# 10XGenomics/lariat

Hardware: AMD Instinct MI355X
Metric: read-pairs/sec aligned to hg38 (per-barcode align loop: SMEM seeding + SW + RFA/MAPQ on device); synthetic hg38-scale reference (higher is better)
Workload: dtype u64/i32 (FM-index + integer DP), f64 (RFA scores)

## Files before the change

include/lariat_hip.h:

```cpp
#ifndef LARIAT_HIP_H
#define LARIAT_HIP_H

#include <stddef.h>
#include <stdint.h>

#ifdef __cplusplus
extern "C" {
#endif

#define LH_ABI_VERSION 11

#define LH_OK 0
#define LH_E_ARG 1
#define LH_E_IO 2
#define LH_E_HIP 3
#define LH_E_CAPACITY 4
#define LH_E_NODEVICE 5
#define LH_E_LIMIT 6

#define LH_MAX_READ_LEN 250

typedef struct lh_index lh_index;
typedef struct lh_context lh_context;

typedef struct lh_opts {
    int32_t abi_version;
    int32_t a, b, o_del, e_del, o_ins, e_ins;
    int32_t pen_unpaired, pen_clip5, pen_clip3;
    int32_t w, zdrop, T;
    int32_t min_seed_len, min_chain_weight, max_chain_extend;
    float split_factor;
    int32_t split_width, max_occ, max_chain_gap, max_ins;
    float mask_level, drop_ratio, XA_drop_ratio, mask_level_redun;
    float mapQ_coef_len;
    int32_t max_mem_intv, max_matesw;
    int32_t pes_low, pes_high;
    int32_t rescue_score_delta;
    int32_t rescue_max_hits;
    int32_t aln_score_delta;
    double improper_pair_penalty;
    double genome_length;
    int32_t run_inference;
    uint32_t flags;
} lh_opts;

#define LH_F_NO_SWEEP_FILTER 1u
#define LH_F_EXT_WAVE 16u
#define LH_F_EXT_SERIAL 32u
#define LH_F_P2_TASKS 128u
#define LH_F_RESCUE_FULL 256u
#define LH_F_SEED_LANE 512u
#define LH_F_TAIL_PASSES 1024u
#define LH_F_RFA_SLAB 2048u
#define LH_F_P2_SCAN 4096u
#define LH_F_P3_LAST 8192u
#define LH_F_CHAIN_WAVE 64u

typedef struct lh_index_opts {
    int32_t abi_version;
    int32_t sa_intv;
    int32_t sb_shift;
    int32_t no_kmer_table;
    int32_t no_unique_runs;
    int32_t no_sweep_filter;
    int32_t build_chunk_log2;
    int32_t ktree_levels;
} lh_index_opts;
void lh_index_opts_init(lh_index_opts* io);

typedef struct lh_context_opts {
    int32_t abi_version;
    int32_t smem_grid;
    int32_t aln_grid;
    int32_t rfa_grid;
    int32_t rfa_slab_kb;
    int32_t lanes;
    int32_t big_slots;
    int32_t rfa_tier_kb[2];
// ... 139 lines not shown
int lh_result_download_end(lh_context* ctx, lh_result** out);
int lh_batch_stage_slot(lh_context* ctx, int32_t slot, const lh_batch* batch);
void* lh_host_alloc(size_t bytes);
void lh_host_free(void* p);
int lh_result_download(lh_context* ctx, lh_result** out);
void lh_result_free(lh_result* r);

typedef struct lh_round_info {
    int32_t n_rounds;
    int32_t max_barcode;
    const int32_t* first_barcode;
    const int64_t* round_seeds;
    const int64_t* round_need_bytes;
    int64_t need_bytes;
    int64_t budget_bytes;
    int64_t max_barcode_need_bytes;
} lh_round_info;
int lh_last_rounds(lh_context* ctx, int32_t lane, lh_round_info* out);

int lh_last_rfa_classes(lh_context* ctx, int64_t* out );

int lh_last_p2_calls(lh_context* ctx, int64_t* out );

int lh_last_fin_list(lh_context* ctx, int32_t* out, int64_t cap, int64_t* n);

int lh_last_timings(lh_context* ctx, int32_t* n, const char* const** names, const float** ms);

int lh_stage_dump_resident(lh_context* ctx, const lh_opts* opts, lh_stage_dump** out);
void lh_stage_dump_free(lh_stage_dump* d);

int lh_get_seq(const lh_index* idx, int32_t rid, int64_t start, int64_t end, int32_t reversed, char* out );

int lh_device_memory(int device, int64_t* free_bytes, int64_t* total_bytes);
int lh_diag_random_read(int device, int64_t table_bytes, int32_t granule_bytes, int64_t n_access, double* gbps, double* ms);

int lh_diag_valu_rate(int device, int32_t op, int32_t waves_per_simd, int32_t iters, double* out, int32_t n_out);

int lh_diag_rescue_sw(int device, int32_t n_cases, const int32_t* q_off, const uint8_t* q, const int32_t* t_off, const uint8_t* t, int32_t full, int32_t weaken, int32_t* out);

int lh_diag_index_check(const lh_index* idx, uint64_t stride, uint64_t* n_checked, uint64_t* n_bad_order, uint64_t* n_bad_lf);

int lh_diag_index_digest(const lh_index* idx, uint64_t* lcp_digest, uint64_t* ktree_digest, int32_t* ktree_levels);

int lh_synth_genome(uint64_t seed, double gc, int64_t l_pac, uint8_t* pac, int32_t threads);
int lh_synth_write_fastq9(const char* path, const uint8_t* seq, const int64_t* seq_off, const int32_t* bc_pair_off, int32_t n_barcodes, int64_t first_barcode,
                          int32_t trim, int32_t gz_level, uint64_t seed, const int32_t* truth_rid, const int64_t* truth_pos1, const int64_t* truth_pos2);
// ... 65 lines not shown
```

lariat_amd/capi.py:

```python
import ctypes as C
import os

import numpy as np

_HERE = os.path.dirname(os.path.abspath(__file__))
LIB_PATH = os.environ.get("LARIAT_HIP_LIB") or os.path.join(_HERE, "_build", "liblariat_hip.so")

LH_OK = 0
LH_ABI_VERSION = 11
LH_E_ARG, LH_E_IO, LH_E_HIP, LH_E_CAPACITY, LH_E_NODEVICE, LH_E_LIMIT = 1, 2, 3, 4, 5, 6
LH_REC_DEBUG_TAGS = 1
LH_F_NO_SWEEP_FILTER, LH_F_EXT_WAVE, LH_F_EXT_SERIAL, LH_F_CHAIN_WAVE, LH_F_P2_TASKS, LH_F_RESCUE_FULL, LH_F_SEED_LANE, LH_F_TAIL_PASSES, LH_F_RFA_SLAB, LH_F_P2_SCAN, LH_F_P3_LAST = 1, 16, 32, 64, 128, 256, 512, 1024, 2048, 4096, 8192
LH_MAX_READ_LEN = 250

c_i32p = C.POINTER(C.c_int32)
c_i64p = C.POINTER(C.c_int64)
c_u8p = C.POINTER(C.c_uint8)
c_u32p = C.POINTER(C.c_uint32)
c_u64p = C.POINTER(C.c_uint64)
c_f64p = C.POINTER(C.c_double)


class LhOpts(C.Structure):
    _fields_ = [
        ("abi_version", C.c_int32),
        ("a", C.c_int32), ("b", C.c_int32), ("o_del", C.c_int32), ("e_del", C.c_int32), ("o_ins", C.c_int32), ("e_ins", C.c_int32),
        ("pen_unpaired", C.c_int32), ("pen_clip5", C.c_int32), ("pen_clip3", C.c_int32),
        ("w", C.c_int32), ("zdrop", C.c_int32), ("T", C.c_int32),
        ("min_seed_len", C.c_int32), ("min_chain_weight", C.c_int32), ("max_chain_extend", C.c_int32),
        ("split_factor", C.c_float),
        ("split_width", C.c_int32), ("max_occ", C.c_int32), ("max_chain_gap", C.c_int32), ("max_ins", C.c_int32),
        ("mask_level", C.c_float), ("drop_ratio", C.c_float), ("XA_drop_ratio", C.c_float), ("mask_level_redun", C.c_float),
        ("mapQ_coef_len", C.c_float),
        ("max_mem_intv", C.c_int32), ("max_matesw", C.c_int32),
        ("pes_low", C.c_int32), ("pes_high", C.c_int32),
# ... 241 lines not shown
    L.lh_records_free.argtypes = [C.c_void_p]
    L.lh_records_free.restype = None
    L.lh_name_seed.argtypes = [C.c_char_p, C.c_int64]
    L.lh_name_seed.restype = C.c_uint64
    L.lh_index_resample_sa.argtypes = [C.c_void_p, C.c_int32]
    L.lh_index_resample_sa.restype = C.c_int
    L.lh_index_sa_interval.argtypes = [C.c_void_p]
    L.lh_index_sa_interval.restype = C.c_int32
    L.lh_index_free.argtypes = [C.c_void_p]
    L.lh_index_build.argtypes = [C.c_char_p, C.c_int32, C.POINTER(C.c_char_p), C.POINTER(c_u8p), c_i64p, C.c_int32]
    L.lh_context_create.argtypes = [C.c_void_p, C.c_int64, C.POINTER(LhContextOpts), C.POINTER(C.c_void_p)]
    L.lh_context_free.argtypes = [C.c_void_p]
    L.lh_align_barcodes.argtypes = [C.c_void_p, C.POINTER(LhOpts), C.POINTER(LhBatch), C.POINTER(C.POINTER(LhResult))]
    L.lh_batch_upload.argtypes = [C.c_void_p, C.POINTER(LhBatch)]
    L.lh_align_resident.argtypes = [C.c_void_p, C.POINTER(LhOpts)]
    L.lh_batch_upload_slot.argtypes = [C.c_void_p, C.c_int32, C.POINTER(LhBatch)]
    L.lh_batch_select.argtypes = [C.c_void_p, C.c_int32]
    L.lh_result_download.argtypes = [C.c_void_p, C.POINTER(C.POINTER(LhResult))]
    L.lh_result_free.argtypes = [C.POINTER(LhResult)]
    L.lh_last_timings.argtypes = [C.c_void_p, c_i32p, C.POINTER(C.POINTER(C.c_char_p)), C.POINTER(C.POINTER(C.c_float))]
    L.lh_last_rounds.argtypes = [C.c_void_p, C.c_int32, C.POINTER(LhRoundInfo)]
    L.lh_last_rfa_classes.argtypes = [C.c_void_p, C.POINTER(C.c_int64)]
    L.lh_last_p2_calls.argtypes = [C.c_void_p, C.POINTER(C.c_int64)]
    L.lh_stage_dump_resident.argtypes = [C.c_void_p, C.POINTER(LhOpts), C.POINTER(C.POINTER(LhStageDump))]
    L.lh_stage_dump_free.argtypes = [C.POINTER(LhStageDump)]
    L.lh_get_seq.argtypes = [C.c_void_p, C.c_int32, C.c_int64, C.c_int64, C.c_int32, C.c_char_p]
    L.lh_device_memory.argtypes = [C.c_int, C.POINTER(C.c_int64), C.POINTER(C.c_int64)]
    L.lh_diag_random_read.argtypes = [C.c_int, C.c_int64, C.c_int32, C.c_int64, C.POINTER(C.c_double), C.POINTER(C.c_double)]
    L.lh_diag_rescue_sw.argtypes = [C.c_int, C.c_int32, c_i32p, c_u8p, c_i32p, c_u8p, C.c_int32, C.c_int32, c_i32p]
    L.lh_diag_valu_rate.argtypes = [C.c_int, C.c_int32, C.c_int32, C.c_int32, C.POINTER(C.c_double), C.c_int32]
    return L


class LhError(RuntimeError):
    def __init__(self, code, msg):
        super().__init__("liblariat_hip error %d: %s" % (code, msg))
        self.code = code


class Library:

    def __init__(self, path=None):
        path = path or LIB_PATH
        if not os.path.exists(path):
            raise RuntimeError("%s not built: run __graft_entry__.build(); there is no CPU fallback" % path)
        self.path = path
# ... 437 lines not shown
        names = C.POINTER(C.c_char_p)()
        ms = C.POINTER(C.c_float)()
        self.lib.check(self.lib.L.lh_last_timings(self.h, C.byref(n), C.byref(names), C.byref(ms)))
        return [(names[i].decode(), float(ms[i])) for i in range(n.value)]

    def rounds(self, lane=0):
        ri = LhRoundInfo()
        self.lib.check(self.lib.L.lh_last_rounds(self.h, int(lane), C.byref(ri)))
        n = int(ri.n_rounds)
        return dict(n_rounds=n, first_barcode=_view(ri.first_barcode, n + 1 if n else 0, np.int32), round_seeds=_view(ri.round_seeds, n, np.int64),
                    round_need_bytes=_view(ri.round_need_bytes, n, np.int64), need_bytes=int(ri.need_bytes), budget_bytes=int(ri.budget_bytes),
                    max_barcode=int(ri.max_barcode), max_barcode_need_bytes=int(ri.max_barcode_need_bytes))

    def rfa_classes(self):
        out = (C.c_int64 * 4)()
        self.lib.check(self.lib.L.lh_last_rfa_classes(self.h, out))
        return dict(big=int(out[0]), rest=int(out[1]), small=int(out[2]), turned_away=int(out[3]))

    def p2_calls(self):
        out = (C.c_int64 * 4)()
        self.lib.check(self.lib.L.lh_last_p2_calls(self.h, out))
        return dict(dropped=int(out[0]), probed=int(out[1]), unprobed=int(out[2]), shares=int(out[3]))

    def fin_list(self):
        L = self.lib.L
        L.lh_last_fin_list.argtypes = [C.c_void_p, c_i32p, C.c_int64, C.POINTER(C.c_int64)]
        n = C.c_int64()
        self.lib.check(L.lh_last_fin_list(self.h, None, 0, C.byref(n)))
        out = np.zeros(max(int(n.value), 1), dtype=np.int32)
        self.lib.check(L.lh_last_fin_list(self.h, out.ctypes.data_as(c_i32p), len(out), C.byref(n)))
        return np.sort(out[:int(n.value)])

    def stage_dump(self, batch=None, opts=None):
        opts = opts or self.lib.opts()
        if batch is not None:
            self.upload(batch)
        d = C.POINTER(LhStageDump)()
        self.lib.check(self.lib.L.lh_stage_dump_resident(self.h, C.byref(opts), C.byref(d)))
        out = StageDump(d.contents)
        self.lib.L.lh_stage_dump_free(d)
        return out


_lib = None


# ... 167 lines not shown
                return
            yield b
            if b.at_eof:
                return

    def close(self):
        if self.h:
            self.lib.L.lh_ingest_close(self.h)
            self.h = None

    def __del__(self):
        try:
            self.close()
        except Exception:
            pass


EXPORTED_SYMBOLS = [
    "lh_last_error", "lh_device_count", "lh_opts_init", "lh_index_load", "lh_index_from_arrays", "lh_index_contigs", "lh_index_l_pac",
    "lh_index_resample_sa", "lh_index_sa_interval",
    "lh_ingest_open", "lh_ingest_next", "lh_ingest_batch_free", "lh_ingest_close", "lh_name_seed",
    "lh_records_text", "lh_records_text_ex", "lh_records_free", "lh_bam_open", "lh_bam_append", "lh_bam_set_flags", "lh_bam_close",
    "lh_index_free", "lh_index_build", "lh_context_create", "lh_context_free", "lh_align_barcodes", "lh_batch_upload", "lh_align_resident",
    "lh_result_download", "lh_result_free", "lh_last_timings", "lh_last_rounds", "lh_last_rfa_classes", "lh_last_p2_calls", "lh_last_fin_list", "lh_stage_dump_resident", "lh_stage_dump_free", "lh_get_seq", "lh_device_memory", "lh_diag_gosort", "lh_diag_gosort_split", "lh_diag_bitonic", "lh_diag_introsort", "lh_diag_random_read", "lh_diag_valu_rate", "lh_diag_rescue_sw", "lh_diag_go_rand", "lh_diag_rescue_dedup",
    "lh_index_opts_init", "lh_context_opts_init", "lh_index_build_device", "lh_index_export", "lh_index_save", "lh_synth_genome", "lh_synth_reads", "lh_synth_write_fastq9", "lh_diag_index_check", "lh_batch_upload_slot", "lh_batch_select", "lh_bam_concat", "lh_reference_pack", "lh_index_set_holes", "lh_diag_index_digest", "lh_index_set_alt", "lh_index_alt", "lh_bam_set_level", "lh_bam_timings", "lh_result_download_begin", "lh_result_download_end", "lh_batch_stage_slot", "lh_host_alloc", "lh_host_free",
    "lh_bgzf_create", "lh_bgzf_free", "lh_bgzf_compress", "lh_bgzf_bound", "lh_bgzf_timings", "lh_bam_set_device",
    "lh_bam_set_device_records", "lh_bam_records_timings", "lh_diag_format_f6",
    "lh_bam_append_resident",
]
```

lariat_amd/csrc/k_smem4.h:

```cpp
#pragma once
#ifndef LH_K1_SLAB_CHUNK
#define LH_K1_SLAB_CHUNK 4
#endif
#include "lh_dev.h"
static_assert((LH_MAXLEN + 2) % LH_K1_SLAB_CHUNK == 0, "a lane's list of LH_MAXLEN + 2 entries is a whole number of chunks");
#define LH_K1_LDS_BUDGET 10240
#ifndef LH_K1_QW_SMALL
#define LH_K1_QW_SMALL 24
#endif
#ifdef LH_K1_RING
#define LH_K1_RING_OF(qw_) (LH_K1_RING)
#else
#define LH_K1_RING_OF(qw_) ((LH_K1_LDS_BUDGET - (qw_) * 256) / 2048)
#endif
static_assert(LH_K1_QW_SMALL >= 1 && LH_K1_QW_SMALL <= 32, "the small query staging holds at most the full query");

struct __attribute__((aligned(16))) PEnt { u64 lo, hi; };
#define LH_M40 0xffffffffffull
__device__ __forceinline__ PEnt pe_pack(u64 x0, u64 x1, u64 x2, int info) {
    PEnt e;
    e.lo = x0 | (x2 << 40);
    e.hi = x1 | ((x2 >> 24) << 40) | ((u64)(uint32_t)info << 49);
    return e;
}
// ... 119 lines not shown
                    }
                    rs.x = bnd; rs.Pk = P; rs.pk = bnd | 2 << 8 | (bnd + 1) << 16;
                    n_ext = e1; n_exec = e2; n_kt = 1;
                }
            }
        }
        if (on >= 0) n_intv[r] = on;
        if (on >= 0 && rs.x >= len) status[r] = 0;
        else { resume[r] = rs; listed = 1; }
    }
    const u64 lm = __ballot(listed);
    if (lm) {
        int basep = 0;
        if (lane == 0) basep = atomicAdd(todo_count, (int32_t)__popcll(lm));
        basep = wave_readlane(basep, 0);
        if (listed) todo[basep + lanes_below(lm, lane)] = r;
    }
    if (ctr) {
        unsigned t1 = (unsigned)wave_sum_i32((int)n_ext), t2 = (unsigned)wave_sum_i32((int)n_exec), t3 = (unsigned)wave_sum_i32((int)n_kt);
        if (lane == 0 && t1) { atomicAdd(&LH_CTR(ctr)->n_ext, (u64)t1); atomicAdd(&LH_CTR(ctr)->n_ext_exec[0], (u64)t2); atomicAdd(&LH_CTR(ctr)->n_ktree[0], (u64)t3); }
    }
}

struct K1Big { const int32_t* list; const int32_t* count; const int32_t* slot; DIntv* slab; union { const K1Resume* resume; int32_t* p2_cnt; }; };
#define LH_P2E_READ ((1ull << 27) - 1)
#define LH_P2E_SHARE (1ull << 27)
#define LH_P2E_TASK 28
#define LH_P2E_XM 28
#define LH_P2E_MIN 36
#define LH_P2E_PBITS 40
#define LH_P2E_UNPROBED (1ull << 59)
#define LH_P2_MAX_MIN_INTV 15
static_assert(LH_BLOOM_K <= 19 && LH_MAXLEN < 256, "a call entry: 8 bits of position, 19 of probe");
#define K1T_OCC 0
#define K1T_TREE 1
#define K1T_BLOOM1 2
#define K1T_BLOOM2 3
#define K1T_REPT 4
#define K1T_PLCP 5
#define K1T_TEXT 6
#define K1T_SA 7
#define K1T_ISA 8
#define K1T_SLAB_R 9
#define K1T_SLAB_W 10
#define K1T_INTV_W 11
#define K1T_READS 12
// ... 1350 lines not shown
```

lariat_amd/csrc/lh_host.inc:

```
#include <math.h>
#include <stdlib.h>
#include <stdio.h>
#include <string.h>

#include <algorithm>
#include <array>
#include <functional>
#include <memory>
#include <mutex>
#include <string>
#include <vector>
#include <deque>
#include <map>

#include "../../include/lariat_hip.h"
#include "k_smem4.h"
#include "k_chain_lane.h"
#include "k_chain_cl.h"
#include "k_rfa.h"
#include "k_rescue3.h"
#include "k_rounds.h"
#include "lh_result_cols.h"

static void lh_print_wd(const int32_t* d_wd) {
// ... 46 lines not shown
    hipStream_t dl_stream = nullptr, up_stream = nullptr;
    hipEvent_t ev_pack = nullptr, ev_dl = nullptr;
    bool dl_pending = false, dl_split = false; std::function<int(lh_result**)> dl_finish;
    int sel_slot = 0;
    HostPeek* h_peek = nullptr;
    bool rfa_merge_big = false;
    i64 rfa_cls[4] = {0, 0, 0, 0};
    bool ext_hint_valid = false;
    hipEvent_t ev_fork = nullptr, ev_join[3] = {nullptr, nullptr, nullptr};
    i64 cap_pairs = 0, cap_reads = 0, cap_bases = 0, pool_cap = 0, regpool_cap = 0, cap_bc = 0;
    DevGroup mem, seed_mem, cand_mem, big_mem, rjob_mem, pack_mem, tier_mem[2], round_mem;
    void free_device() {
        for (DevGroup* g : {&mem, &seed_mem, &cand_mem, &big_mem, &rjob_mem, &pack_mem, &tier_mem[0], &tier_mem[1], &round_mem}) g->release();
        for (DevBatch& sl : slots) sl.mem.release();
        for (void* q : free_later) hipFree(q);
        free_later.clear();
    }
    int grid_smem4 = 0; PEnt* d_slab4 = nullptr; K1Counters* d_next_read = nullptr;
    BatchView b;
    uint32_t* d_seq4 = nullptr;
    const uint32_t* q4 = nullptr;
    DIntv* d_intv = nullptr; DIntv* d_big_slab = nullptr; int32_t *d_big_slot = nullptr, *d_big_list = nullptr; K1BigCounts* d_big_count = nullptr; int big_cap = 0, big_base = 0;
    K1Resume* d_k1_resume = nullptr; int32_t* d_k1_todo = nullptr;
    u64* d_p2_tasks = nullptr; P2Calls* d_p2_calls = nullptr;
    i64 p2_cls[4] = {0, 0, 0, 0};
    int32_t *d_n_intv = nullptr, *d_seed_cnt = nullptr, *d_l_rep = nullptr, *d_status = nullptr;
    int32_t* d_fin_list = nullptr;
    i64* d_seed_off = nullptr; DSeed* d_seeds = nullptr; int32_t *d_s_rid = nullptr, *d_s_next = nullptr, *d_ord = nullptr, *d_srt = nullptr;
    DChainTmp* d_ct = nullptr; DChain* d_chains = nullptr; DSeed* d_cseeds = nullptr; int32_t* d_n_chains = nullptr;
    DCounters* d_ctr = nullptr; i64* d_tile_sum = nullptr;
    int32_t* d_wd = nullptr;
    i64* d_reg_off = nullptr; DReg* d_regs = nullptr; int32_t* d_n_regs = nullptr; i64* d_chain_rmax = nullptr;
    DReg* d_regs_tmp = nullptr;
    int32_t* d_ia = nullptr;
    int32_t *d_ext_defer = nullptr, *d_ext_heavy = nullptr, *d_ext_jlist = nullptr, *d_ext_jkey = nullptr, *d_ext_jorder = nullptr; ExtSt* d_ext_st = nullptr;
    DExtJobs* d_ext_jobs = nullptr; DExtJobs* d_ext_jobs2 = nullptr;
    int32_t* d_ext_long = nullptr;
    int32_t* d_ext_u = nullptr;
    int32_t* d_best = nullptr;
    uint8_t* d_reg_clean = nullptr;
    uint8_t* d_dd_done = nullptr;
    int32_t* d_dd_list = nullptr;
    int32_t* d_rnj = nullptr; i64* d_rjob_off = nullptr; RMeta* d_rmeta = nullptr; int32_t* d_rkeys = nullptr; int32_t* d_rheavy = nullptr;
    RJob* d_rjobs = nullptr; int32_t *d_rorder = nullptr, *d_rorder2 = nullptr; i64 rjob_cap = 0;
    i64 cand_cap = 0; int grid_aln = 0; DCand R; uint8_t* d_zpool = nullptr;
    int32_t *d_aln_r = nullptr, *d_aln_ci = nullptr; AlnCounts* d_aln_count = nullptr;
// ... 152 lines not shown
    HIPCHK(hipStreamCreate(&c->stream));
    for (int i = 0; i < 3; ++i) { HIPCHK(hipStreamCreate(&c->aux[i])); HIPCHK(hipEventCreateWithFlags(&c->ev_join[i], hipEventDisableTiming)); }
    HIPCHK(hipEventCreateWithFlags(&c->ev_fork, hipEventDisableTiming));
    {
        int lo = 0, hi = 0;
        HIPCHK(hipDeviceGetStreamPriorityRange(&lo, &hi));
        HIPCHK(hipStreamCreateWithPriority(&c->dl_stream, hipStreamNonBlocking, lo));
        HIPCHK(hipStreamCreateWithPriority(&c->up_stream, hipStreamNonBlocking, lo));
    }
    HIPCHK(hipHostMalloc((void**)&c->h_peek, sizeof(HostPeek), hipHostMallocDefault));
    HIPCHK(hipEventCreateWithFlags(&c->ev_pack, hipEventDisableTiming)); HIPCHK(hipEventCreateWithFlags(&c->ev_dl, hipEventDisableTiming));
    i64 N = c->cap_reads;
    DevGroup& g = c->mem;
    DALLOC(g, c->d_seq4, c->cap_bases / 8 + 16); HIPCHK(hipMemset(c->d_seq4, 0x44, 16));
    {
        lh_context::DevBatch& s0 = c->slots.emplace_back();
        DALLOC(s0.mem, s0.v.seq, c->cap_bases + 64); DALLOC(s0.mem, s0.v.seq_off, N + 1); DALLOC(s0.mem, s0.v.name_seed, max_pairs);
        DALLOC(s0.mem, s0.v.bc_pair_off, c->cap_bc + 1); DALLOC(s0.mem, s0.v.bc_do_rfa, c->cap_bc);
        DALLOC(s0.mem, s0.v.cen_start, idx->names.size()); DALLOC(s0.mem, s0.v.cen_end, idx->names.size());
        select_slot(c, s0);
    }
    DALLOC(g, c->d_intv, N * LH_MAX_INTV); DALLOC(g, c->d_n_intv, N);
    c->big_cap = c->co.big_slots > 0 ? c->co.big_slots : LH_MAX_INTV < 16 ? (int)N : (int)(N / 256 > 64 ? N / 256 : 64);
    DALLOC(g, c->d_k1_resume, N); DALLOC(g, c->d_k1_todo, N); DALLOC(g, c->d_p2_tasks, (size_t)LH_P2_SPLIT * N); DALLOC(g, c->d_p2_calls, LH_CTR_SLOTS);
    DALLOC(c->big_mem, c->d_big_slab, (size_t)c->big_cap * 2 * LH_BIG_INTV); DALLOC(g, c->d_big_slot, N); DALLOC(c->big_mem, c->d_big_list, c->big_cap); DALLOC(g, c->d_big_count, 1);
    DALLOC(g, c->d_seed_cnt, N); DALLOC(g, c->d_l_rep, N); DALLOC(g, c->d_status, N); DALLOC(g, c->d_fin_list, N);
    {
        int want = c->co.smem_grid;
        i64 need = (c->cap_reads + 63) / 64;
        c->grid_smem4 = (int)(need < want ? need : want);
        DALLOC(g, c->d_slab4, (size_t)c->grid_smem4 * 64 * 2 * (LH_MAXLEN + 2));
        DALLOC(g, c->d_next_read, 1);
    }
    DALLOC(g, c->d_seed_off, N + 1); DALLOC(g, c->d_n_chains, N);
    if (c->co.seed_budget_kb < 0 || pool_cap_limit(c) < 1)
        return set_err(LH_E_ARG, "lh_context_opts.seed_budget_kb = " + std::to_string(c->co.seed_budget_kb) + ": the rescue slots of " + std::to_string(max_pairs) +
                                     " pairs alone take " + std::to_string((seed_need(c, 0) >> 10) + 1) + " KiB");
    { int rc = alloc_seed_pools(c, first_pool_cap(c)); if (rc) return rc; }
    DALLOC(g, c->d_ctr, LH_CTR_SLOTS);
    DALLOC(g, c->d_wd, LH_WD_SLOTS);
    HIPCHK(hipMemset(c->d_wd, 0, LH_WD_SLOTS * sizeof(int32_t)));
    { int rc = stage2_alloc(c); if (rc) return rc; }
    for (int i = 0; i <= LH_NSTAGE; ++i) HIPCHK(hipEventCreate(&c->ev[i]));
    guard.c = nullptr;
    *out = c;
    return LH_OK;
}
// ... 174 lines not shown
static inline int ext_long_min(int N);
struct K1Tail {
    bool probe;
    bool tasks;
    bool list;
    bool p3_lock;
    bool p3_counts;
    bool fused;
};
static K1Tail k1_tail_plan(const lh_context* c, const DOpts& o, int N, bool packed_reads) {
    K1Tail t;
    const bool list_ok = N < (1 << 27);
    t.probe = list_ok && !(c->flags & (LH_F_P2_TASKS | LH_F_P2_SCAN)) && o.split_width < LH_P2_MAX_MIN_INTV;
    t.p3_lock = o.max_mem_intv > 0 && packed_reads;
    t.p3_counts = t.p3_lock && !(c->flags & LH_F_SEED_LANE);
#ifdef LH_K1_TRACE
    t.probe = t.p3_counts = false;
#endif
    t.tasks = list_ok && !t.probe && ((c->flags & LH_F_P2_TASKS) || (c->ext_hint_valid && c->h_peek->prev_wave_reads >= ext_long_min(N)));
    t.list = t.probe || t.tasks;
    t.fused = t.probe && t.p3_counts && !(c->flags & LH_F_P3_LAST);
    return t;
}
static int run_front(lh_context* c, const DOpts& o, int& t) {
    int N = c->b.n_reads;
    const DIndex& ix = c->idx->d;
    HIPCHK(hipMemsetAsync(c->d_ctr, 0, sizeof(DCounters) * LH_CTR_SLOTS, c->stream));
    const uint32_t* q4 = nullptr;
    if (ix.tn) {
        LH_LAUNCH(k_pack_reads, 4096, 256, c->stream, (const uint8_t*)c->b.seq, c->b.n_bases, c->d_seq4 + 2);
        q4 = c->d_seq4 + 2;
    }
    c->q4 = q4;
    DIndex ix4 = ix;
    if (c->flags & LH_F_NO_SWEEP_FILTER) ix4.bloom1 = ix4.bloom2 = nullptr;
    {
        const int g4 = (N + 63) / 64 < c->grid_smem4 ? (N + 63) / 64 : c->grid_smem4;
        HIPCHK(hipMemsetAsync(c->d_next_read, 0, sizeof(K1Counters), c->stream));
        K1Big nobig; nobig.list = nullptr; nobig.count = nullptr; nobig.slot = nullptr; nobig.slab = nullptr; nobig.resume = nullptr;
        K1Big first = nobig; first.list = c->d_k1_todo; first.count = &c->d_next_read->n_todo; first.resume = c->d_k1_resume;
        const int g3 = (N + 63) / 64 < 2 * c->grid_smem4 ? (N + 63) / 64 : 2 * c->grid_smem4;
        T_BEGIN("k_smem4");
        LH_LAUNCH(k_smem_first, (N + 255) / 256, 256, c->stream, ix4, o, N, q4, (const i64*)c->b.seq_off, c->d_intv, c->d_n_intv, c->d_status, c->d_k1_resume, c->d_k1_todo, &c->d_next_read->n_todo, c->d_ctr);
#ifdef LH_K1_TRACE
        K1Trace trace;
        { int rc = k1_trace_begin(c, trace, g4); if (rc) return rc; }
#endif
        const bool qw_small = c->b.max_len <= 8 * LH_K1_QW_SMALL;
        if (qw_small) smem_pass<1, false, LH_K1_QW_SMALL>(c, ix4, o, N, g4, first);
        else smem_pass<1, false>(c, ix4, o, N, g4, first);
        T_END();
#ifdef LH_K1_TRACE
        { int rc = k1_trace_replay(c, trace, N, g4); if (rc) return rc; }
#endif
        HIPCHK(hipMemsetAsync(c->d_p2_calls, 0, sizeof(P2Calls) * LH_CTR_SLOTS, c->stream));
        const K1Tail tail = k1_tail_plan(c, o, N, q4 != nullptr);
        K1Big p2 = nobig;
        if (tail.list) { p2.list = (const int32_t*)c->d_p2_tasks; p2.count = &c->d_next_read->n_p2_tasks; p2.slot = c->d_k1_todo; }
        if (tail.fused) {
            T_BEGIN("k_smem4_p3");
            LH_LAUNCH(k_p23_lock, (N + 255) / 256, 256, c->stream, ix4, o, N, (const uint8_t*)c->b.seq, q4, (const i64*)c->b.seq_off, c->d_intv, c->d_n_intv, c->d_ctr, c->d_seed_cnt, c->d_p2_tasks,
                      &c->d_next_read->n_p2_tasks, c->d_k1_todo, c->d_p2_calls);
            T_END();
            T_BEGIN("k_smem4_p2");
            p2.p2_cnt = c->d_seed_cnt;
            if (qw_small) smem_pass<2, false, LH_K1_QW_SMALL>(c, ix4, o, N, g4, p2);
            else smem_pass<2, false>(c, ix4, o, N, g4, p2);
            LH_LAUNCH(k_p2_close, (N + 255) / 256, 256, c->stream, N, c->d_n_intv, c->d_status, c->d_seed_cnt, c->d_l_rep, c->d_fin_list, &c->d_next_read->n_fin);
            T_END();
#ifdef LH_P3_KINDS
// ... 260 lines not shown
            rc = pipe_download(c, &res);
            c->ran = false;
            if (rc) rc = set_err(rc, "round " + std::to_string(r) + " of " + std::to_string(n_rounds) + " (its reads start at read " + std::to_string(2 * (i64)p0) + " of the batch): " + g_err);
        }
        if (!rc) rc = merge_into(acc, res);
        if (rc) {
            const std::string why = g_err;
            quiesce(c);
            if (acc) lh_result_free(acc);
            return set_err(rc, why);
        }
    }
    c->round_result = acc;
    R.n_rounds = (int)n_rounds;
    c->n_t = sums.n;
    for (int i = 0; i < sums.n; ++i) { c->tnames[i] = sums.names[i]; c->tms[i] = sums.ms[i]; }
    return LH_OK;
}

static int pipe_align(lh_context* c, const lh_opts* opts) {
    if (!c || !opts) return set_err(LH_E_ARG, "lh_align_resident: null argument");
    if (!c->resident) return set_err(LH_E_ARG, "no batch resident: call lh_batch_upload first");
    if (opts->abi_version != LH_ABI_VERSION) return set_err(LH_E_ARG, "lh_opts.abi_version does not match LH_ABI_VERSION (use lh_opts_init)");
    if (opts->flags & ~(LH_F_NO_SWEEP_FILTER | LH_F_EXT_WAVE | LH_F_EXT_SERIAL | LH_F_CHAIN_WAVE | LH_F_P2_TASKS | LH_F_RESCUE_FULL | LH_F_SEED_LANE | LH_F_TAIL_PASSES | LH_F_RFA_SLAB | LH_F_P2_SCAN | LH_F_P3_LAST)) return set_err(LH_E_ARG, "lh_opts.flags: unknown bit set");
    HIPCHK(hipSetDevice(c->idx->device));
    {
        std::vector<void*> fl;
        { std::lock_guard<std::mutex> g(c->slot_mu); fl.swap(c->free_later); }
        for (void* q : fl) hipFree(q);
    }
    if (c->round_result) { lh_result_free(c->round_result); c->round_result = nullptr; }
    c->rounds.clear();
    c->ran = false;
    if (!c->pool_cap) { int rc = alloc_seed_pools(c, first_pool_cap(c)); if (rc) return rc; }
    if (!c->cand_cap) { int rc = alloc_cand_pools(c, first_cand_cap(c)); if (rc) return rc; }
    DOpts o = to_dopts(opts);
    o.wd = c->d_wd;
    c->flags = opts->flags;
    int t = 0;
    int rc = run_front(c, o, t);
    const bool in_rounds = rc == LH_NEED_ROUNDS;
    if (in_rounds) rc = align_rounds(c, o, t);
    else if (!rc) rc = stage2_run(c, o, t);
    if (rc) { quiesce(c); return rc; }
    if (!in_rounds) {
        HIPCHK(hipEventRecord(c->ev[t], c->stream));
        HIPCHK(hipStreamSynchronize(c->stream));
// ... 114 lines not shown
```

lariat_amd/csrc/lh_lanes.inc:

```
#include <atomic>
#include <thread>

#define LH_MAX_LANES 4

int lh_context_create(lh_index* idx, int64_t max_pairs, const lh_context_opts* co, lh_context** out) {
    const int lanes = co && co->lanes ? co->lanes : 1;
    if (lanes < 1 || lanes > LH_MAX_LANES) return set_err(LH_E_ARG, "lh_context_opts.lanes must be 1 .. 4");
    lh_context* c = nullptr;
    int rc = pipe_create(idx, max_pairs, co, &c);
    if (rc) return rc;
    for (int k = 1; k < lanes && max_pairs >= 2 * lanes; ++k) {
        lh_context_opts c2 = *co;
        c2.lanes = 1;
        {
            const int g = (c2.rfa_grid > 0 ? c2.rfa_grid : 4096) / lanes;
            c2.rfa_grid = g > 1024 ? g : 1024;
        }
        int64_t cap = max_pairs / lanes + 30000 < max_pairs ? max_pairs / lanes + 30000 : max_pairs;
        lh_context* p = nullptr;
        rc = pipe_create(idx, cap, &c2, &p);
        if (rc) { lh_context_free(c); return rc; }
        c->more.push_back(p);
    }
    *out = c;
// ... 123 lines not shown
        R.have_max = true;
    }
    const int32_t b0 = lane && lanes_split(c) ? c->slot_cut[(size_t)c->cur_slot][(size_t)lane - 1] : 0;
    if (b0 && R.first_bc[0] == 0) { for (int32_t& b : R.first_bc) b += b0; R.max_bc += b0; }
    out->n_rounds = R.n_rounds; out->max_barcode = (int32_t)R.max_bc;
    out->first_barcode = R.first_bc.data(); out->round_seeds = R.seeds.data(); out->round_need_bytes = R.need.data();
    out->need_bytes = seed_need(p, R.total_seeds); out->budget_bytes = R.budget; out->max_barcode_need_bytes = seed_need(p, R.max_bc_seeds);
    return LH_OK;
}

int lh_last_rfa_classes(lh_context* c, int64_t* out) {
    if (!c || !out) return set_err(LH_E_ARG, "lh_last_rfa_classes: null argument");
    if (!c->ran_inference) return set_err(LH_E_ARG, "lh_last_rfa_classes: call lh_align_resident with run_inference first");
    for (int i = 0; i < 4; ++i) out[i] = c->rfa_cls[i];
    return LH_OK;
}

int lh_last_p2_calls(lh_context* c, int64_t* out) {
    if (!c || !out) return set_err(LH_E_ARG, "lh_last_p2_calls: null argument");
    for (int i = 0; i < 4; ++i) out[i] = c->p2_cls[i];
    return LH_OK;
}

int lh_last_fin_list(lh_context* c, int32_t* out, int64_t cap, int64_t* n) {
    if (!c || !n || cap < 0 || (cap && !out)) return set_err(LH_E_ARG, "lh_last_fin_list: null argument");
    if (!c->d_fin_list || !c->d_next_read) return set_err(LH_E_ARG, "lh_last_fin_list: call lh_align_resident or lh_stage_dump_resident first");
    HIPCHK(hipSetDevice(c->idx->device));
    HIPCHK(hipStreamSynchronize(c->stream));
    int32_t n_fin = 0;
    HIPCHK(hipMemcpy(&n_fin, &c->d_next_read->n_fin, sizeof n_fin, hipMemcpyDeviceToHost));
    *n = n_fin;
    const int64_t k = n_fin < cap ? n_fin : cap;
    if (k > 0) HIPCHK(hipMemcpy(out, c->d_fin_list, (size_t)k * sizeof(int32_t), hipMemcpyDeviceToHost));
    return LH_OK;
}

static int merge_into(lh_result*& acc, lh_result* part) {
    if (!acc) { acc = part; return LH_OK; }
    lh_result* m = nullptr;
    const int rc = merge_results(acc, part, &m);
    lh_result_free(acc); lh_result_free(part);
    acc = m;
    return rc;
}
static int merge_results(lh_result* a, lh_result* b, lh_result** out) {
    const size_t Ca = (size_t)a->n_cand, Cb = (size_t)b->n_cand;
// ... 118 lines not shown
```

lariat_amd/csrc/lh_workspace.h:

```cpp
#pragma once
#include <stddef.h>
#include <vector>

template <class T> static int dalloc(T** p, size_t n) {
    hipError_t e = hipMalloc((void**)p, (n ? n : 1) * sizeof(T));
    if (e != hipSuccess) { *p = nullptr; (void)hipGetLastError(); return set_err(LH_E_HIP, std::string("hipMalloc of ") + std::to_string((n ? n : 1) * sizeof(T)) + " bytes: " + hipGetErrorString(e)); }
    return LH_OK;
}

struct DevGroup {
    std::vector<void**> held;
    DevGroup() = default;
    DevGroup(const DevGroup&) = delete;
    DevGroup& operator=(const DevGroup&) = delete;
    ~DevGroup() { release(); }
    template <class T> int alloc(T*& p, size_t n) {
        int rc = dalloc(&p, n);
        if (rc) release(); else held.push_back((void**)&p);
        return rc;
    }
    void release() { for (void** q : held) { hipFree(*q); *q = nullptr; } held.clear(); }
    void release_to(std::vector<void*>& later) { for (void** q : held) { if (*q) later.push_back(*q); *q = nullptr; } held.clear(); }
};
#define DALLOC(g, p, n) do { int rc_ = (g).alloc(p, (size_t)(n)); if (rc_) return rc_; } while (0)

struct BatchView {
    uint8_t* seq = nullptr; i64* seq_off = nullptr;
    u64* name_seed = nullptr;
    int32_t* bc_pair_off = nullptr; uint8_t* bc_do_rfa = nullptr;
    i64 *cen_start = nullptr, *cen_end = nullptr;
    int n_pairs = 0, n_reads = 0, n_bc = 0; bool has_cen = false; i64 n_bases = 0;
    int max_len = LH_MAXLEN;
};

struct K1Counters {
    int32_t pass[3];
    int32_t big_pass[3];
    int32_t n_todo;
    int32_t n_p2_tasks;
    int32_t n_fin;
};
static_assert(sizeof(K1Counters) == 9 * sizeof(int32_t) && offsetof(K1Counters, big_pass) == 3 * sizeof(int32_t) && sizeof(K1Counters::big_pass) == 3 * sizeof(int32_t),
              "the second chance's counters are cleared as one range");
struct K1BigCounts {
    int32_t listed;
    int32_t asked;
};
static_assert(offsetof(K1BigCounts, listed) == 0 && offsetof(K1BigCounts, asked) == sizeof(int32_t) && sizeof(K1BigCounts) == 2 * sizeof(int32_t), "k_big_collect: count[0], count[1]");
struct AlnCounts {
    int32_t flat;
    int32_t grp16;
    int32_t grp32;
    int32_t full;
};
static_assert(offsetof(AlnCounts, flat) == 0 && sizeof(AlnCounts) == 4 * sizeof(int32_t), "K7 clears all four, the download the first");
struct RfaCounters {
    int32_t next;
    int32_t n_ovf;
    int32_t last_next;
    int32_t heavy_pairs;
    int32_t heavy_reads;
    int32_t post_next;
    int32_t post_n_ovf;
    int32_t post_last_next;
    struct Tier {
// ... 93 lines not shown
```

Baseline: 56.32 million.

## Settle near-exact K1 reads by direct reference comparison before SMEM pass

Adds a k_smem_settle kernel that runs before the first SMEM pass. For each pending read it compares the query directly against the reference at the resumed position. When there are few mismatches, the PLCP check shows the exact segments are unique, and no bloom-filter k-mer hit exists around the mismatches, it writes the exact-match intervals directly and removes the read from the todo list. Only the remaining reads go to the costly FM-index SMEM pass. This adds one extra kernel launch, reads of plcp and bloom, and relies on heuristics that must stay equivalent to full SMEM output.

```diff
diff --git a/include/lariat_hip.h b/include/lariat_hip.h
--- a/include/lariat_hip.h
+++ b/include/lariat_hip.h
@@ -8,7 +8,7 @@
 extern "C" {
 #endif
 
-#define LH_ABI_VERSION 11
+#define LH_ABI_VERSION 12
 
 #define LH_OK 0
 #define LH_E_ARG 1
@@ -54,6 +54,7 @@
 #define LH_F_RFA_SLAB 2048u
 #define LH_F_P2_SCAN 4096u
 #define LH_F_P3_LAST 8192u
+#define LH_F_K1_NO_SETTLE 16384u
 #define LH_F_CHAIN_WAVE 64u
 
 typedef struct lh_index_opts {
@@ -239,6 +240,8 @@
 
 int lh_last_p2_calls(lh_context* ctx, int64_t* out );
 
+int lh_last_k1_settled(lh_context* ctx, int64_t* out );
+
 int lh_last_fin_list(lh_context* ctx, int32_t* out, int64_t cap, int64_t* n);
 
 int lh_last_timings(lh_context* ctx, int32_t* n, const char* const** names, const float** ms);
diff --git a/lariat_amd/capi.py b/lariat_amd/capi.py
--- a/lariat_amd/capi.py
+++ b/lariat_amd/capi.py
@@ -7,10 +7,10 @@
 LIB_PATH = os.environ.get("LARIAT_HIP_LIB") or os.path.join(_HERE, "_build", "liblariat_hip.so")
 
 LH_OK = 0
-LH_ABI_VERSION = 11
+LH_ABI_VERSION = 12
 LH_E_ARG, LH_E_IO, LH_E_HIP, LH_E_CAPACITY, LH_E_NODEVICE, LH_E_LIMIT = 1, 2, 3, 4, 5, 6
 LH_REC_DEBUG_TAGS = 1
-LH_F_NO_SWEEP_FILTER, LH_F_EXT_WAVE, LH_F_EXT_SERIAL, LH_F_CHAIN_WAVE, LH_F_P2_TASKS, LH_F_RESCUE_FULL, LH_F_SEED_LANE, LH_F_TAIL_PASSES, LH_F_RFA_SLAB, LH_F_P2_SCAN, LH_F_P3_LAST = 1, 16, 32, 64, 128, 256, 512, 1024, 2048, 4096, 8192
+LH_F_NO_SWEEP_FILTER, LH_F_EXT_WAVE, LH_F_EXT_SERIAL, LH_F_CHAIN_WAVE, LH_F_P2_TASKS, LH_F_RESCUE_FULL, LH_F_SEED_LANE, LH_F_TAIL_PASSES, LH_F_RFA_SLAB, LH_F_P2_SCAN, LH_F_P3_LAST, LH_F_K1_NO_SETTLE = 1, 16, 32, 64, 128, 256, 512, 1024, 2048, 4096, 8192, 16384
 LH_MAX_READ_LEN = 250
 
 c_i32p = C.POINTER(C.c_int32)
@@ -298,6 +298,7 @@
     L.lh_last_rounds.argtypes = [C.c_void_p, C.c_int32, C.POINTER(LhRoundInfo)]
     L.lh_last_rfa_classes.argtypes = [C.c_void_p, C.POINTER(C.c_int64)]
     L.lh_last_p2_calls.argtypes = [C.c_void_p, C.POINTER(C.c_int64)]
+    L.lh_last_k1_settled.argtypes = [C.c_void_p, C.POINTER(C.c_int64)]
     L.lh_stage_dump_resident.argtypes = [C.c_void_p, C.POINTER(LhOpts), C.POINTER(C.POINTER(LhStageDump))]
     L.lh_stage_dump_free.argtypes = [C.POINTER(LhStageDump)]
     L.lh_get_seq.argtypes = [C.c_void_p, C.c_int32, C.c_int64, C.c_int64, C.c_int32, C.c_char_p]
@@ -781,6 +782,11 @@
         self.lib.check(self.lib.L.lh_last_p2_calls(self.h, out))
         return dict(dropped=int(out[0]), probed=int(out[1]), unprobed=int(out[2]), shares=int(out[3]))
 
+    def k1_settled(self):
+        out = (C.c_int64 * 5)()
+        self.lib.check(self.lib.L.lh_last_k1_settled(self.h, out))
+        return dict(listed=int(out[0]), settled=int(out[1]), too_many=int(out[2]), not_unique=int(out[3]), window=int(out[4]))
+
     def fin_list(self):
         L = self.lib.L
         L.lh_last_fin_list.argtypes = [C.c_void_p, c_i32p, C.c_int64, C.POINTER(C.c_int64)]
@@ -994,7 +1000,7 @@
     "lh_ingest_open", "lh_ingest_next", "lh_ingest_batch_free", "lh_ingest_close", "lh_name_seed",
     "lh_records_text", "lh_records_text_ex", "lh_records_free", "lh_bam_open", "lh_bam_append", "lh_bam_set_flags", "lh_bam_close",
     "lh_index_free", "lh_index_build", "lh_context_create", "lh_context_free", "lh_align_barcodes", "lh_batch_upload", "lh_align_resident",
-    "lh_result_download", "lh_result_free", "lh_last_timings", "lh_last_rounds", "lh_last_rfa_classes", "lh_last_p2_calls", "lh_last_fin_list", "lh_stage_dump_resident", "lh_stage_dump_free", "lh_get_seq", "lh_device_memory", "lh_diag_gosort", "lh_diag_gosort_split", "lh_diag_bitonic", "lh_diag_introsort", "lh_diag_random_read", "lh_diag_valu_rate", "lh_diag_rescue_sw", "lh_diag_go_rand", "lh_diag_rescue_dedup",
+    "lh_result_download", "lh_result_free", "lh_last_timings", "lh_last_rounds", "lh_last_rfa_classes", "lh_last_p2_calls", "lh_last_k1_settled", "lh_last_fin_list", "lh_stage_dump_resident", "lh_stage_dump_free", "lh_get_seq", "lh_device_memory", "lh_diag_gosort", "lh_diag_gosort_split", "lh_diag_bitonic", "lh_diag_introsort", "lh_diag_random_read", "lh_diag_valu_rate", "lh_diag_rescue_sw", "lh_diag_go_rand", "lh_diag_rescue_dedup",
     "lh_index_opts_init", "lh_context_opts_init", "lh_index_build_device", "lh_index_export", "lh_index_save", "lh_synth_genome", "lh_synth_reads", "lh_synth_write_fastq9", "lh_diag_index_check", "lh_batch_upload_slot", "lh_batch_select", "lh_bam_concat", "lh_reference_pack", "lh_index_set_holes", "lh_diag_index_digest", "lh_index_set_alt", "lh_index_alt", "lh_bam_set_level", "lh_bam_timings", "lh_result_download_begin", "lh_result_download_end", "lh_batch_stage_slot", "lh_host_alloc", "lh_host_free",
     "lh_bgzf_create", "lh_bgzf_free", "lh_bgzf_compress", "lh_bgzf_bound", "lh_bgzf_timings", "lh_bam_set_device",
     "lh_bam_set_device_records", "lh_bam_records_timings", "lh_diag_format_f6",
diff --git a/lariat_amd/csrc/k_smem4.h b/lariat_amd/csrc/k_smem4.h
--- a/lariat_amd/csrc/k_smem4.h
+++ b/lariat_amd/csrc/k_smem4.h
@@ -165,6 +165,124 @@
     }
 }
 
+
+#ifndef LH_K1_SETTLE_MAXDIFF
+#define LH_K1_SETTLE_MAXDIFF 3
+#endif
+static_assert(LH_K1_SETTLE_MAXDIFF >= 1 && LH_K1_SETTLE_MAXDIFF <= 4 && LH_MAXLEN < 256, "the differences' positions: a byte each in one word");
+#ifndef LH_SETTLE_BATCH
+#define LH_SETTLE_BATCH LH_BLOOM_K
+#endif
+__device__ __forceinline__ uint32_t dev_code8(uint32_t w) {
+    w &= 0x33333333u;
+    w = (w | w >> 2) & 0x0f0f0f0fu; w = (w | w >> 4) & 0x00ff00ffu; w = (w | w >> 8) & 0xffffu;
+    return w;
+}
+__device__ __forceinline__ u64 dev_settle_key(u64 lo, uint32_t hi, int t) { return (t ? lo >> (2 * t) | (u64)hi << (64 - 2 * t) : lo) & ((1ull << (2 * LH_BLOOM_K)) - 1); }
+__global__ void __launch_bounds__(256) k_smem_settle(DIndex ix, DOpts o, const uint32_t* __restrict__ q4, const i64* __restrict__ seq_off, DIntv* __restrict__ intv_out, int32_t* __restrict__ n_intv,
+                                                      int32_t* __restrict__ status, const K1Resume* __restrict__ resume, const int32_t* __restrict__ todo, const int32_t* __restrict__ todo_count,
+                                                      int32_t* __restrict__ todo2, int32_t* __restrict__ counts) {
+    const int k = blockIdx.x * blockDim.x + threadIdx.x, lane = LANE();
+    int r = -1, why = -1;
+    if (k < *todo_count) {
+        r = todo[k];
+        const K1Resume rs = resume[r];
+        const i64 off = seq_off[r], P = rs.Pk;
+        const int len = (int)(seq_off[r + 1] - off);
+        why = 0;
+        if (P >= 0 && len >= o.min_seed_len && len <= LH_MAXLEN && P + len <= (i64)ix.seq_len && rs.x > 0 && rs.x < len) {
+            uint32_t dpos = 0;
+            int nd = 0, nonbase = 0;
+            for (int i = rs.x; i < len && nd <= LH_K1_SETTLE_MAXDIFF; i += 8) {
+                const uint32_t qw = dev_nib8(q4, off + i), tw = dev_nib8(ix.tn, P + i);
+                const uint32_t m = len - i < 8 ? (1u << (4 * (len - i))) - 1u : ~0u;
+                nonbase |= (qw & 0xccccccccu & m) != 0;
+                uint32_t x = (qw ^ tw) & m;
+                while (x) {
+                    const int b = (__ffs((int)x) - 1) >> 2;
+                    if (nd < 4) dpos |= (uint32_t)(i + b) << (8 * nd);
+                    ++nd;
+                    x &= ~(0xfu << (4 * b));
+                }
+            }
+#define SETTLE_M(j_) ((int)((dpos >> (8 * (j_))) & 0xff))
+#define SETTLE_S(j_) (SETTLE_M(j_) + 1)
+#define SETTLE_E(j_) ((j_) + 1 < nd ? SETTLE_M((j_) + 1) : len)
+            if (nd > LH_K1_SETTLE_MAXDIFF) why = 1;
+            else if (!nonbase && nd > 0) {
+                why = 4;
+#ifndef LH_SETTLE_WEAK_PLCP
+                uint32_t lc[LH_K1_SETTLE_MAXDIFF];
+#pragma unroll
+                for (int j = 0; j < LH_K1_SETTLE_MAXDIFF; ++j) lc[j] = j < nd && SETTLE_E(j) - SETTLE_S(j) >= o.min_seed_len ? ix.plcp[P + SETTLE_S(j)] : 0u;
+#pragma unroll
+                for (int j = 0; j < LH_K1_SETTLE_MAXDIFF; ++j)
+                    if (j < nd && SETTLE_E(j) - SETTLE_S(j) >= o.min_seed_len && (int)lc[j] >= SETTLE_E(j) - SETTLE_S(j)) why = 2;
+#endif
+                int done = -1;
+                for (int j = 0; j < nd && why == 4; ++j) {
+                    const int m = SETTLE_M(j);
+                    int w0 = m - (LH_BLOOM_K - 1), w1 = m < len - LH_BLOOM_K ? m : len - LH_BLOOM_K;
+                    if (w0 < 0) w0 = 0;
+                    if (w0 <= done) w0 = done + 1;
+                    done = w1 > done ? w1 : done;
+#ifdef LH_SETTLE_WEAK_WINDOW
+                    --w1;
+#endif
+                    if (w0 > w1) continue;
+                    const u64 lo = (u64)dev_code8(dev_nib8(q4, off + w0)) | (u64)dev_code8(dev_nib8(q4, off + w0 + 8)) << 16 | (u64)dev_code8(dev_nib8(q4, off + w0 + 16)) << 32 |
+                                   (u64)dev_code8(dev_nib8(q4, off + w0 + 24)) << 48;
+                    const uint32_t hi = dev_code8(dev_nib8(q4, off + w0 + 32));
+                    for (int t0 = 0; t0 <= w1 - w0 && why == 4; t0 += LH_SETTLE_BATCH) {
+                        u64 bw[LH_SETTLE_BATCH];
+#pragma unroll
+                        for (int u = 0; u < LH_SETTLE_BATCH; ++u) {
+                            bw[u] = 0;
+                            if (t0 + u <= w1 - w0) {
+                                uint32_t w_; u64 mask_;
+                                dev_bloom_slot(dev_settle_key(lo, hi, t0 + u), ix.bloom1_words, &w_, &mask_);
+                                bw[u] = ix.bloom1[w_];
+                            }
+                        }
+#pragma unroll
+                        for (int u = 0; u < LH_SETTLE_BATCH; ++u) {
+                            if (t0 + u <= w1 - w0) {
+                                uint32_t w_; u64 mask_;
+                                dev_bloom_slot(dev_settle_key(lo, hi, t0 + u), ix.bloom1_words, &w_, &mask_);
+                                if ((bw[u] & mask_) == mask_) why = 3;
+                            }
+                        }
+                    }
+                }
+                if (why == 4) {
+                    DIntv* const out = intv_out + (size_t)r * LH_MAX_INTV;
+                    int on = n_intv[r], ovf = 0;
+                    for (int j = 0; j < nd; ++j) {
+                        const int s = SETTLE_S(j), e = SETTLE_E(j);
+                        if (e - s < o.min_seed_len) continue;
+                        if (on >= LH_MAX_INTV) ovf = 1;
+                        else { DIntv mm; mm.x0 = LH_POSF | (u64)(P + s); mm.x1 = 0; mm.x2 = 1; mm.info = (u64)s << 32 | (u64)e; out[on++] = mm; }
+                    }
+                    n_intv[r] = on;
+                    status[r] = ovf ? LH_ST_INTV_OVERFLOW : 0;
+                }
+            }
+#undef SETTLE_M
+#undef SETTLE_S
+#undef SETTLE_E
+        }
+    }
+    const int listed = why >= 0 && why < 4;
+    const u64 lm = __ballot(listed);
+    if (lm) {
+        int basep = 0;
+        if (lane == 0) basep = atomicAdd(&counts[0], (int32_t)__popcll(lm));
+        basep = wave_readlane(basep, 0);
+        if (listed) todo2[basep + lanes_below(lm, lane)] = r;
+        const int c1 = (int)__popcll(__ballot(why == 1)), c2 = (int)__popcll(__ballot(why == 2)), c3 = (int)__popcll(__ballot(why == 3));
+        if (lane == 0) { if (c1) atomicAdd(&counts[1], c1); if (c2) atomicAdd(&counts[2], c2); if (c3) atomicAdd(&counts[3], c3); }
+    }
+}
 struct K1Big { const int32_t* list; const int32_t* count; const int32_t* slot; DIntv* slab; union { const K1Resume* resume; int32_t* p2_cnt; }; };
 #define LH_P2E_READ ((1ull << 27) - 1)
 #define LH_P2E_SHARE (1ull << 27)
diff --git a/lariat_amd/csrc/lh_host.inc b/lariat_amd/csrc/lh_host.inc
--- a/lariat_amd/csrc/lh_host.inc
+++ b/lariat_amd/csrc/lh_host.inc
@@ -92,6 +92,8 @@
     const uint32_t* q4 = nullptr;
     DIntv* d_intv = nullptr; DIntv* d_big_slab = nullptr; int32_t *d_big_slot = nullptr, *d_big_list = nullptr; K1BigCounts* d_big_count = nullptr; int big_cap = 0, big_base = 0;
     K1Resume* d_k1_resume = nullptr; int32_t* d_k1_todo = nullptr;
+    int32_t* d_k1_todo2 = nullptr; bool k1_settle_ran = false;
+    bool k1_ran = false;
     u64* d_p2_tasks = nullptr; P2Calls* d_p2_calls = nullptr;
     i64 p2_cls[4] = {0, 0, 0, 0};
     int32_t *d_n_intv = nullptr, *d_seed_cnt = nullptr, *d_l_rep = nullptr, *d_status = nullptr;
@@ -290,7 +292,7 @@
     }
     DALLOC(g, c->d_intv, N * LH_MAX_INTV); DALLOC(g, c->d_n_intv, N);
     c->big_cap = c->co.big_slots > 0 ? c->co.big_slots : LH_MAX_INTV < 16 ? (int)N : (int)(N / 256 > 64 ? N / 256 : 64);
-    DALLOC(g, c->d_k1_resume, N); DALLOC(g, c->d_k1_todo, N); DALLOC(g, c->d_p2_tasks, (size_t)LH_P2_SPLIT * N); DALLOC(g, c->d_p2_calls, LH_CTR_SLOTS);
+    DALLOC(g, c->d_k1_resume, N); DALLOC(g, c->d_k1_todo, N); DALLOC(g, c->d_k1_todo2, N); DALLOC(g, c->d_p2_tasks, (size_t)LH_P2_SPLIT * N); DALLOC(g, c->d_p2_calls, LH_CTR_SLOTS);
     DALLOC(c->big_mem, c->d_big_slab, (size_t)c->big_cap * 2 * LH_BIG_INTV); DALLOC(g, c->d_big_slot, N); DALLOC(c->big_mem, c->d_big_list, c->big_cap); DALLOC(g, c->d_big_count, 1);
     DALLOC(g, c->d_seed_cnt, N); DALLOC(g, c->d_l_rep, N); DALLOC(g, c->d_status, N); DALLOC(g, c->d_fin_list, N);
     {
@@ -511,6 +513,16 @@
     t.fused = t.probe && t.p3_counts && !(c->flags & LH_F_P3_LAST);
     return t;
 }
+static bool k1_settle_on(const lh_context* c, const DIndex& ix4, const DOpts& o, const uint32_t* q4) {
+#ifdef LH_K1_TRACE
+    (void)c; (void)ix4; (void)o; (void)q4;
+    return false;
+#else
+    const int ktl = ix4.ktree ? ix4.ktree_levels : 0;
+    const bool first_can = ix4.isa && ix4.tn && q4 && ix4.bloom1 && ktl >= 2 && ktl <= 16 && ktl < LH_BLOOM_K && o.min_seed_len >= LH_BLOOM_K;
+    return first_can && ix4.plcp && !(c->flags & LH_F_K1_NO_SETTLE);
+#endif
+}
 static int run_front(lh_context* c, const DOpts& o, int& t) {
     int N = c->b.n_reads;
     const DIndex& ix = c->idx->d;
@@ -535,6 +547,12 @@
         K1Trace trace;
         { int rc = k1_trace_begin(c, trace, g4); if (rc) return rc; }
 #endif
+        c->k1_settle_ran = k1_settle_on(c, ix4, o, q4); c->k1_ran = true;
+        if (c->k1_settle_ran) {
+            LH_LAUNCH(k_smem_settle, (N + 255) / 256, 256, c->stream, ix4, o, q4, (const i64*)c->b.seq_off, c->d_intv, c->d_n_intv, c->d_status, (const K1Resume*)c->d_k1_resume, (const int32_t*)c->d_k1_todo,
+                      (const int32_t*)&c->d_next_read->n_todo, c->d_k1_todo2, c->d_next_read->settle);
+            first.list = c->d_k1_todo2; first.count = &c->d_next_read->settle[0];
+        }
         const bool qw_small = c->b.max_len <= 8 * LH_K1_QW_SMALL;
         if (qw_small) smem_pass<1, false, LH_K1_QW_SMALL>(c, ix4, o, N, g4, first);
         else smem_pass<1, false>(c, ix4, o, N, g4, first);
@@ -841,7 +859,7 @@
     if (!c || !opts) return set_err(LH_E_ARG, "lh_align_resident: null argument");
     if (!c->resident) return set_err(LH_E_ARG, "no batch resident: call lh_batch_upload first");
     if (opts->abi_version != LH_ABI_VERSION) return set_err(LH_E_ARG, "lh_opts.abi_version does not match LH_ABI_VERSION (use lh_opts_init)");
-    if (opts->flags & ~(LH_F_NO_SWEEP_FILTER | LH_F_EXT_WAVE | LH_F_EXT_SERIAL | LH_F_CHAIN_WAVE | LH_F_P2_TASKS | LH_F_RESCUE_FULL | LH_F_SEED_LANE | LH_F_TAIL_PASSES | LH_F_RFA_SLAB | LH_F_P2_SCAN | LH_F_P3_LAST)) return set_err(LH_E_ARG, "lh_opts.flags: unknown bit set");
+    if (opts->flags & ~(LH_F_NO_SWEEP_FILTER | LH_F_EXT_WAVE | LH_F_EXT_SERIAL | LH_F_CHAIN_WAVE | LH_F_P2_TASKS | LH_F_RESCUE_FULL | LH_F_SEED_LANE | LH_F_TAIL_PASSES | LH_F_RFA_SLAB | LH_F_P2_SCAN | LH_F_P3_LAST | LH_F_K1_NO_SETTLE)) return set_err(LH_E_ARG, "lh_opts.flags: unknown bit set");
     HIPCHK(hipSetDevice(c->idx->device));
     {
         std::vector<void*> fl;
diff --git a/lariat_amd/csrc/lh_lanes.inc b/lariat_amd/csrc/lh_lanes.inc
--- a/lariat_amd/csrc/lh_lanes.inc
+++ b/lariat_amd/csrc/lh_lanes.inc
@@ -169,6 +169,18 @@
     return LH_OK;
 }
 
+int lh_last_k1_settled(lh_context* c, int64_t* out) {
+    if (!c || !out) return set_err(LH_E_ARG, "lh_last_k1_settled: null argument");
+    if (!c->d_next_read || !c->k1_ran) return set_err(LH_E_ARG, "lh_last_k1_settled: call lh_align_resident or lh_stage_dump_resident first");
+    HIPCHK(hipSetDevice(c->idx->device));
+    HIPCHK(hipStreamSynchronize(c->stream));
+    K1Counters k;
+    HIPCHK(hipMemcpy(&k, c->d_next_read, sizeof k, hipMemcpyDeviceToHost));
+    out[0] = k.n_todo; out[1] = c->k1_settle_ran ? k.n_todo - k.settle[0] : 0;
+    for (int i = 0; i < 3; ++i) out[2 + i] = c->k1_settle_ran ? k.settle[1 + i] : 0;
+    return LH_OK;
+}
+
 int lh_last_fin_list(lh_context* c, int32_t* out, int64_t cap, int64_t* n) {
     if (!c || !n || cap < 0 || (cap && !out)) return set_err(LH_E_ARG, "lh_last_fin_list: null argument");
     if (!c->d_fin_list || !c->d_next_read) return set_err(LH_E_ARG, "lh_last_fin_list: call lh_align_resident or lh_stage_dump_resident first");
diff --git a/lariat_amd/csrc/lh_workspace.h b/lariat_amd/csrc/lh_workspace.h
--- a/lariat_amd/csrc/lh_workspace.h
+++ b/lariat_amd/csrc/lh_workspace.h
@@ -39,8 +39,9 @@
     int32_t n_todo;
     int32_t n_p2_tasks;
     int32_t n_fin;
+    int32_t settle[4];
 };
-static_assert(sizeof(K1Counters) == 9 * sizeof(int32_t) && offsetof(K1Counters, big_pass) == 3 * sizeof(int32_t) && sizeof(K1Counters::big_pass) == 3 * sizeof(int32_t),
+static_assert(sizeof(K1Counters) == 13 * sizeof(int32_t) && offsetof(K1Counters, big_pass) == 3 * sizeof(int32_t) && sizeof(K1Counters::big_pass) == 3 * sizeof(int32_t),
               "the second chance's counters are cleared as one range");
 struct K1BigCounts {
     int32_t listed;
```

Result: no change. 56.80 million (median of 6 runs) (+0.9%).
